# josl/kmerjs

Measured on AMD Instinct MI355X. Metric: k-mers/sec + distinct-kmers/sec, k=16 150bp synthetic FASTQ, 1/2/4/8 GPU, higher is better.
Workload: dtype u8; 1 GPU; C2: 10000000 synthetic 150bp reads per GPU, k=16, prefix 'ATGAC'; reads_per_gpu=10000000, mode=ordered (reference Map insertion order), k=16, prefix=ATGAC, bytes_per_gpu=3170000000, pipeline=off (steps in sequence), parallelism=dp1 (one GPU; no collective), backend=none

## Files before the change

### kmerjs_amd/csrc/kmer_kernels.hip

```cpp
#include "kmer_device.hpp"

#include <algorithm>
#include <cstring>

namespace kmerhip {

__device__ __forceinline__ uint32_t align4(uint32_t hi, uint32_t lo, uint32_t sel) {
    return __builtin_amdgcn_alignbyte(hi, lo, sel);
}

__device__ __forceinline__ void set_info(unsigned int *err, unsigned int bit) {
    if (!(__hip_atomic_load(err, __ATOMIC_RELAXED, __HIP_MEMORY_SCOPE_AGENT) & bit)) atomicOr(err, bit);
}

__device__ __forceinline__ uint32_t not_nl_bits(uint32_t x) {
    return ((x ^ 0x0A0A0A0Au) + 0x7F7F7F7Fu) & 0x80808080u;
}

__device__ __forceinline__ uint32_t not_nl_bits_xad(uint32_t x, uint32_t k0a, uint32_t k7f) {
    uint32_t r;
    asm("v_xad_u32 %0, %1, %2, %3" : "=v"(r) : "v"(x), "v"(k0a), "s"(k7f));
    return r & 0x80808080u;
}

__device__ __forceinline__ uint8_t comp_byte(uint8_t c) {
    return c == 'A' ? 'T' : c == 'T' ? 'A' : c == 'G' ? 'C' : c == 'C' ? 'G' : c;
}

__device__ __forceinline__ uint64_t lb_load(unsigned long long *p) {
    return __hip_atomic_load(p, __ATOMIC_RELAXED, __HIP_MEMORY_SCOPE_AGENT);
}
__device__ __forceinline__ void lb_store(unsigned long long *p, uint64_t v) {
    __hip_atomic_store(p, (unsigned long long)v, __ATOMIC_RELAXED, __HIP_MEMORY_SCOPE_AGENT);
}

constexpr uint32_t SPIN_LIMIT = 1u << 22;

template <bool SUM>
__device__ uint64_t look_back(unsigned long long *words, uint32_t tile, unsigned int *err) {
    const int lane = threadIdx.x & 63;
    uint64_t acc = 0;
    int64_t top = (int64_t)tile - 1;
    uint32_t spins = 0;
    while (true) {
        int64_t idx = top - lane;
        uint64_t v = 0;
        bool valid = idx >= 0;
        while (true) {
            v = valid ? lb_load(words + idx) : LB_INC;
            bool ready = (v >> 62) != 0;
            if (__all(ready)) break;
            if (++spins > SPIN_LIMIT) {
                if (lane == 0) atomicOr(err, ERR_LOOKBACK_TIMEOUT);
                return acc;
            }
            __builtin_amdgcn_s_sleep(1);
        }
        const uint64_t val = valid ? (v & LB_VAL) : 0;
        const bool inc = (v >> 62) == 2;
        if (SUM) {
            unsigned long long incmask = __ballot(inc);
            int stop = incmask ? __ffsll((long long)incmask) - 1 : 64;
            uint64_t contrib = lane <= stop ? val : 0;
            for (int d = 32; d >= 1; d >>= 1) contrib += __shfl_xor(contrib, d);
            acc += contrib;
            if (incmask) return acc;
        } else {
            unsigned long long hit = __ballot(inc || val != 0);
            if (hit) {
                int stop = __ffsll((long long)hit) - 1;
                return __shfl(val, stop);
            }
        }
        top -= 64;
    }
}

struct TileShared {
    uint32_t tpre[TPB + 1];
    uint32_t wsum[TPB / 64];
    int32_t last_thr;
    uint32_t tile;
    uint64_t line_base;
    uint64_t lnl_before;
    uint64_t lnl_tile;
    int32_t lastpos;
    uint32_t nh;
    uint32_t qn;
    uint32_t more;
    uint32_t q[1024];
};

__device__ __forceinline__ uint32_t nl_before_in_thread(const uint8_t *buf, int thr, int q) {
    const uint32_t *lw = (const uint32_t *)(buf + FH + 64 * thr);
    int n = q - 64 * thr;
    uint32_t c = 0;
#pragma unroll 1
    for (int i = 0; i < 16 && n > 0; ++i, n -= 4) {
        uint32_t z = nl_flags(lw[i]);
        if (n < 4) z &= (1u << (8 * n)) - 1u;
        c += __popc(z);
    }
    return c;
}

__device__ __forceinline__ uint32_t lds_word(const uint8_t *buf, int p) {
    const int a = FH + p;
    const uint32_t *w = (const uint32_t *)(buf + (a & ~3));
    return align4(w[1], w[0], (uint32_t)(a & 3));
}


__device__ __forceinline__ uint64_t revcomp_code(uint64_t x, uint32_t k) {
    x = ~x;
    x = ((x >> 2) & 0x3333333333333333ull) | ((x & 0x3333333333333333ull) << 2);
    x = ((x >> 4) & 0x0F0F0F0F0F0F0F0Full) | ((x & 0x0F0F0F0F0F0F0F0Full) << 4);
    x = __builtin_bswap64(x);
// ... 729 lines not shown
                                                uint32_t *lk, bool *lvalid_out, uint64_t *key_hi) {
    const uint32_t t = r.tile;
    const uint32_t strand = (r.qm >> 14) & 1u;
    const bool exotic = (r.qm >> 15) & 1u;
    const bool lvalid = (r.qm >> 16) & 1u;
    const int q = (int)(r.qm & 0x3FFFu);
    const int s0 = strand ? q + (int)a.plen - (int)a.k : q;
    const uint64_t tile_abs = a.abs_offset + (uint64_t)t * TILE;
    const uint64_t li = pos_lines + tb.cnt + r.c_local;
    const uint64_t lstart = lvalid ? tile_abs + r.lstart : tb.lnl;
    const uint64_t sabs = tile_abs + (uint64_t)(int64_t)s0;
    uint64_t rel = sabs - lstart;
    const bool seq = (li & 3) == 1;
    const uint64_t maxrel = (1ull << a.pbits) - 1ull;
    if (rel > maxrel) {
        if (seq) atomicOr(a.err, ERR_LINE_TOO_LONG);
        rel = maxrel;
    }
    if (li >> (63 - a.pbits)) atomicOr(a.err, ERR_LINE_TOO_LONG);
    const uint64_t order = (li << (a.pbits + 1)) | ((uint64_t)strand << a.pbits) | (strand ? maxrel - rel : rel);
    *order_out = order;
    const uint32_t sp = (uint32_t)(s0 + 64);
    *lk = (r.c_local << 17) | (strand << 16) | (strand ? 0xFFFFu - sp : sp);
    *lvalid_out = lvalid;
    uint64_t key = a.invalid_key;
    *key_hi = a.wide ? a.invalid_key : 0;
    if (a.wide) key = 0;
    if (seq) {
        if (a.packed && !exotic) {
            if (a.k > 32) {
                uint64_t h = code_hi, l = r.code;
                if (strand) revcomp_code128(code_hi, r.code, a.k, &h, &l);
                key = l & a.smask;
                *key_hi = h & a.smask_hi;
            } else {
                key = (strand ? revcomp_code(r.code, a.k) : r.code) & a.smask;
            }
        } else {
            append_record(a.recs, a.rec_count, a.rec_cap, a.err, order, (uint64_t)t * TILE + (uint64_t)(int64_t)s0, a.k,
                          strand);
        }
    }
    return key;
}

__device__ __forceinline__ void place_hit(const HitArgs &a, uint64_t slot, bool cross, uint64_t xi, uint64_t key,
                                          uint64_t key_hi, uint64_t order) {
    if (!cross) {
        if (slot >= a.rcap) {
            atomicOr(a.err, ERR_OVF_OVERFLOW);
            return;
        }
        if (a.rkey32) a.rkey32[slot] = (uint32_t)key;
        else a.rkey[slot] = key;
        if (a.wide) a.rkeyh[slot] = key_hi;
        a.rord[slot] = order;
    } else if (xi < a.xcap) {
        a.xord[xi] = order;
        a.xslot[xi] = (uint32_t)slot;
        if (a.wide) {
            a.xkey[xi] = xi;
            a.xkeyl[xi] = key;
            a.xkeyh[xi] = key_hi;
        } else {
            a.xkey[xi] = key;
        }
    } else {
        atomicOr(a.err, ERR_CROSS_OVERFLOW);
    }
}

constexpr uint32_t HTPW = 4;
constexpr uint32_t HENT = HTPW * HMAX;
template <bool WIDE>
__global__ __launch_bounds__(256) void hit_kernel(HitArgs a) {
    __shared__ uint32_t s_lk[4][HENT];
    __shared__ uint8_t s_x[4][HENT];
    __shared__ uint64_t s_key[4][HENT];
    __shared__ uint64_t s_ord[4][HENT];
    __shared__ uint64_t s_keyh[WIDE ? 4 : 1][WIDE ? HENT : 1];
    const uint32_t wid = threadIdx.x >> 6, lane = threadIdx.x & 63;
    const uint32_t t0 = __builtin_amdgcn_readfirstlane((blockIdx.x * 4 + wid) * HTPW);
    if (t0 >= a.n_tiles) return;
    const unsigned long long ovf = *a.ovf_count;
    const uint64_t pos_lines = a.pos->lines;
    TileSum ts[HTPW], tb[HTPW];
#pragma unroll
    for (uint32_t u = 0; u < HTPW; ++u) {
        const uint32_t t = min(t0 + u, a.n_tiles - 1);
        ts[u] = a.tsum[t];
        tb[u] = a.tscan[t];
    }
    if (ovf > a.ovf_cap) return;
    uint32_t off[HTPW + 1];
    off[0] = 0;
#pragma unroll
    for (uint32_t u = 0; u < HTPW; ++u) off[u + 1] = off[u] + (t0 + u < a.n_tiles ? min(ts[u].nh, (uint32_t)HMAX) : 0u);
    const uint32_t total = off[HTPW];
    for (uint32_t e0 = 0; e0 < total; e0 += 64) {
        const uint32_t e = e0 + lane;
        if (e < total) {
            uint32_t u = 0;
#pragma unroll
            for (uint32_t v = 1; v < HTPW; ++v) u += e >= off[v] ? 1u : 0u;
            const uint32_t i = e - off[u];
            TileSum tsu = ts[0], tbu = tb[0];
#pragma unroll
            for (uint32_t v = 1; v < HTPW; ++v)
                if (u == v) {
                    tsu = ts[v];
                    tbu = tb[v];
                }
            const uint64_t hslot = (uint64_t)(t0 + u) * HMAX + i;
            const HitRec r = a.hits[hslot];
            uint64_t order, kh;
            uint32_t lk;
            bool lvalid;
            const uint64_t key = resolve_hit(a, pos_lines, r, a.k > 32 ? a.hits_hi[hslot] : 0, tbu, &order, &lk, &lvalid,
                                             &kh);
            s_lk[wid][e] = lk;
            s_x[wid][e] = (tsu.nh > (uint32_t)HMAX || !lvalid || r.c_local == (uint32_t)tsu.cnt) ? 1 : 0;
            s_key[wid][e] = key;
            if (WIDE) s_keyh[WIDE ? wid : 0][WIDE ? e : 0] = kh;
            s_ord[wid][e] = order;
        }
    }
    if (!a.packed) return;
    __builtin_amdgcn_fence(__ATOMIC_RELEASE, "workgroup");
    __builtin_amdgcn_wave_barrier();
    for (uint32_t e0 = 0; e0 < total; e0 += 64) {
        const uint32_t e = e0 + lane;
        if (e >= total) continue;
        uint32_t u = 0;
#pragma unroll
        for (uint32_t v = 1; v < HTPW; ++v) u += e >= off[v] ? 1u : 0u;
        uint32_t lo = off[0], hi = off[1], nh = ts[0].nh;
        uint64_t hb = tb[0].nh, xb = tb[0].nx;
#pragma unroll
        for (uint32_t v = 1; v < HTPW; ++v)
            if (u == v) {
                lo = off[v];
                hi = off[v + 1];
                nh = ts[v].nh;
                hb = tb[v].nh;
                xb = tb[v].nx;
            }
        const uint32_t i = e - lo;
        const bool cross = s_x[wid][e] != 0;
        uint32_t rank = i, xr = i;
        if (nh <= (uint32_t)HMAX) {
            const uint32_t lk = s_lk[wid][e];
            rank = 0;
            xr = 0;
            for (uint32_t j = lo; j < hi; ++j) {
                const uint32_t less = s_lk[wid][j] < lk ? 1u : 0u;
                rank += less;
                xr += less & (uint32_t)s_x[wid][j];
            }
        }
        place_hit(a, a.out_base + hb + rank, cross, a.xbase + xb + xr, s_key[wid][e],
                  WIDE ? s_keyh[WIDE ? wid : 0][WIDE ? e : 0] : 0, s_ord[wid][e]);
    }
}

__global__ __launch_bounds__(256) void hit_overflow_kernel(HitArgs a) {
    const uint64_t n = *a.ovf_count <= a.ovf_cap ? *a.ovf_count : 0;
    for (uint64_t i = (uint64_t)blockIdx.x * blockDim.x + threadIdx.x; i < n; i += (uint64_t)gridDim.x * blockDim.x) {
        const HitRec r = a.ovf[i];
        const TileSum tb = a.tscan[r.tile];
        uint64_t order, kh;
        uint32_t lk;
        bool lvalid;
        const uint64_t key = resolve_hit(a, a.pos->lines, r, a.k > 32 ? a.ovf_hi[i] : 0, tb, &order, &lk, &lvalid, &kh);
        if (!a.packed) continue;
        const uint32_t ord = r.qm >> 17;
        place_hit(a, a.out_base + tb.nh + ord, true, a.xbase + tb.nx + ord, key, kh, order);
    }
    __shared__ bool last;
    __syncthreads();
    if (threadIdx.x == 0) {
        __threadfence();
        last = atomicAdd(a.ticket, 1u) == gridDim.x - 1;
    }
    __syncthreads();
    if (!last || threadIdx.x != 0) return;
    __threadfence();
    const uint32_t nt = a.n_tiles;
    StreamPos *pos = (StreamPos *)a.pos;
    pos->lines += a.tscan[nt - 1].cnt + a.tsum[nt - 1].cnt;
    pos->ends_open = (a.len > 0 && a.data[a.len - 1] != '\n') ? 1 : 0;
    *a.ends_open = pos->ends_open;
    *a.chunk_hits = a.tscan[nt - 1].nh + a.tsum[nt - 1].nh;
    *a.chunk_cross = a.tscan[nt - 1].nx + a.tsum[nt - 1].nx;
    *a.ticket = 0;
    if (a.stamp) a.stamp[STAMP_FEED_END] = wall_clock64();
    const uint64_t errw = __hip_atomic_load(a.scal + 5, __ATOMIC_RELAXED, __HIP_MEMORY_SCOPE_AGENT);
    *a.cross_go = ((uint32_t)errw & CROSS_HOST_BITS) ? 0u : 1u;
    __threadfence();
    if (a.host_out) {
        for (int i = 0; i < 8; ++i)
            a.host_out[i] = i == 5 ? errw : __hip_atomic_load(a.scal + i, __ATOMIC_RELAXED, __HIP_MEMORY_SCOPE_AGENT);
        if (a.stamp)
            for (int i = 0; i <= (int)STAMP_FEED_END; ++i)
                a.host_out[TAIL_STAMP + i] = __hip_atomic_load(a.stamp + i, __ATOMIC_RELAXED, __HIP_MEMORY_SCOPE_AGENT);
        __threadfence_system();
        __hip_atomic_store(a.host_out + 9, a.seq, __ATOMIC_RELEASE, __HIP_MEMORY_SCOPE_SYSTEM);
    }
}

__device__ __forceinline__ TileSum ts_shfl_up(const TileSum &v, int d) {
    TileSum r;
    r.cnt = (uint64_t)__shfl_up((unsigned long long)v.cnt, d);
    r.nh = (uint32_t)__shfl_up((int)v.nh, d);
    r.nx = (uint32_t)__shfl_up((int)v.nx, d);
    r.lnl = (uint64_t)__shfl_up((unsigned long long)v.lnl, d);
    return r;
}
__device__ __forceinline__ TileSum ts_zero() {
    TileSum z;
    z.cnt = 0;
    z.nh = 0;
    z.nx = 0;
    z.lnl = 0;
    return z;
}
__device__ __forceinline__ TileSum ts_wave_scan(TileSum v) {
    const int lane = threadIdx.x & 63;
#pragma unroll
    for (int d = 1; d < 64; d <<= 1) {
        const TileSum o = ts_shfl_up(v, d);
        if (lane >= d) v = tile_sum_op(o, v);
    }
    return v;
}
__device__ __forceinline__ TileSum ts_block_scan(TileSum v, TileSum *total) {
    __shared__ TileSum wsum[4];
    const int lane = threadIdx.x & 63, wid = threadIdx.x >> 6;
    const TileSum incl = ts_wave_scan(v);
    if (lane == 63) wsum[wid] = incl;
    __syncthreads();
    TileSum pre = ts_zero(), tot = ts_zero();
#pragma unroll
    for (int w = 0; w < 4; ++w) {
        if (w < wid) pre = tile_sum_op(pre, wsum[w]);
        tot = tile_sum_op(tot, wsum[w]);
    }
    __syncthreads();
    *total = tot;
    const TileSum ex = ts_shfl_up(incl, 1);
    return lane == 0 ? pre : tile_sum_op(pre, ex);
}

__global__ __launch_bounds__(256) void tile_reduce_kernel(const TileSum *in, uint32_t n, TileSum *bsum,
                                                          uint64_t *stamp) {
    stamp_now(stamp, STAMP_SCAN_END);
    const uint32_t base = blockIdx.x * TSCAN_BLOCK;
    TileSum v = ts_zero();
#pragma unroll
    for (uint32_t i = 0; i < TSCAN_BLOCK / 256; ++i) {
        const uint32_t t = base + i * 256 + threadIdx.x;
        if (t < n) v = tile_sum_op(v, in[t]);
    }
    TileSum tot;
    (void)ts_block_scan(v, &tot);
    if (threadIdx.x == 0) bsum[blockIdx.x] = tot;
}

__global__ __launch_bounds__(256) void tile_scan_kernel(const TileSum *in, uint32_t n, const TileSum *bsum,
                                                        uint32_t bsum_scanned, TileSum init, TileSum *out) {
    const uint32_t b = blockIdx.x;
    TileSum pre;
    if (bsum_scanned) {
        pre = tile_sum_op(init, bsum[b]);
    } else {
        TileSum v = ts_zero();
        for (uint32_t j = threadIdx.x; j < b; j += 256) v = tile_sum_op(v, bsum[j]);
        TileSum tot;
        (void)ts_block_scan(v, &tot);
        pre = tile_sum_op(init, tot);
    }
    const uint32_t t0 = b * TSCAN_BLOCK + threadIdx.x * 4;
    TileSum x[4];
    TileSum acc = ts_zero();
#pragma unroll
    for (int i = 0; i < 4; ++i) {
        x[i] = t0 + i < n ? in[t0 + i] : ts_zero();
        acc = tile_sum_op(acc, x[i]);
    }
    TileSum tot;
// ... 999 lines not shown
        HeadRec v;
        v.key = 0;
        v.count = 0;
        if (k != invalid_key && (i == 0 || skey[i - 1] != k)) {
            const uint64_t e = group_end(skey, i, n, k);
            uint64_t cnt = e - i;
            if (rcnt) {
                cnt = 0;
                for (uint64_t j = i; j < e; ++j) cnt += rcnt[srank[j]];
            }
            v.key = k;
            v.count = cnt;
        }
        const uint32_t r = srank[i];
        hrec[r] = v;
        hcnt[r] = v.count ? 1u : 0u;
    }
}

template <typename K>
__global__ __launch_bounds__(256) void heads_sparse_kernel(const K *skey, const uint32_t *srank, uint64_t n,
                                                           K invalid_key, uint32_t *hcnt) {
    for (uint64_t i = (uint64_t)blockIdx.x * blockDim.x + threadIdx.x; i < n; i += (uint64_t)gridDim.x * blockDim.x) {
        const K k = skey[i];
        const bool dp = i > 0 && skey[i - 1] == k;
        const bool dn = i + 1 < n && skey[i + 1] == k;
        if (k != invalid_key && !dp && !dn) continue;
        uint32_t v = 0;
        if (k != invalid_key && !dp) v = (uint32_t)(group_end(skey, i, n, k) - i);
        hcnt[srank[i]] = v;
    }
}

__global__ __launch_bounds__(256) void gather_u64_kernel(const uint64_t *src, const uint32_t *idx, uint64_t n,
                                                         uint64_t *dst) {
    for (uint64_t i = (uint64_t)blockIdx.x * blockDim.x + threadIdx.x; i < n; i += (uint64_t)gridDim.x * blockDim.x)
        dst[i] = src[idx[i]];
}

__global__ __launch_bounds__(256) void cross_wide_fix_kernel(const uint32_t *xslot, uint64_t n, const uint64_t *xkeyl,
                                                             const uint64_t *xkeyh, uint64_t *rkey, uint64_t *rkeyh) {
    for (uint64_t i = (uint64_t)blockIdx.x * blockDim.x + threadIdx.x; i < n; i += (uint64_t)gridDim.x * blockDim.x) {
        const uint32_t sl = xslot[i];
        const uint64_t x = rkey[sl];
        rkey[sl] = xkeyl[x];
        rkeyh[sl] = xkeyh[x];
    }
}

__global__ __launch_bounds__(256) void heads_wide_kernel(const uint64_t *shi, const uint64_t *slo,
                                                         const uint32_t *srank, uint64_t n, uint64_t invalid_hi,
                                                         uint32_t *hcnt) {
    for (uint64_t i = (uint64_t)blockIdx.x * blockDim.x + threadIdx.x; i < n; i += (uint64_t)gridDim.x * blockDim.x) {
        const uint64_t h = shi[i], l = slo[i];
        const bool dp = i > 0 && shi[i - 1] == h && slo[i - 1] == l;
        const bool dn = i + 1 < n && shi[i + 1] == h && slo[i + 1] == l;
        const bool inv = h == invalid_hi;
        if (!inv && !dp && !dn) continue;
        uint32_t v = 0;
        if (!inv && !dp) {
            uint64_t e = i + 1;
            while (e < n && shi[e] == h && slo[e] == l) ++e;
            v = (uint32_t)(e - i);
        }
        hcnt[srank[i]] = v;
    }
}

constexpr uint32_t BKT_EPB = 4096;

__global__ __launch_bounds__(256) void bucket_hist_kernel(const uint32_t *key, uint64_t n, uint32_t invalid,
                                                          uint32_t shift, uint32_t nb, uint32_t nblk,
                                                          uint32_t *H, uint32_t *hcnt, uint64_t *stamp) {
    stamp_now(stamp, STAMP_FINISH_START);
    __shared__ uint32_t hist[BKT_MAX];
    for (uint32_t b = threadIdx.x; b < nb; b += 256) hist[b] = 0;
    __syncthreads();
    const uint64_t base = (uint64_t)blockIdx.x * BKT_EPB;
    for (uint32_t j = 4 * threadIdx.x; j < BKT_EPB; j += 4 * 256) {
        const uint64_t i = base + j;
        if (i + 4 <= n) *(uint4 *)(hcnt + i) = make_uint4(0, 0, 0, 0);
        else for (uint64_t t = i; t < n; ++t) hcnt[t] = 0;
    }
#pragma unroll 4
    for (uint32_t j = threadIdx.x; j < BKT_EPB; j += 256) {
        const uint64_t i = base + j;
        if (i < n) {
            const uint32_t k = key[i];
            if (k != invalid) atomicAdd(&hist[k >> shift], 1u);
        }
    }
    __syncthreads();
    for (uint32_t b = threadIdx.x; b < nb; b += 256) H[(uint64_t)b * nblk + blockIdx.x] = hist[b];
}

__global__ __launch_bounds__(256) void bucket_offsets_kernel(const uint32_t *H, uint32_t nb, uint32_t nblk,
                                                             uint32_t *Hs, uint32_t *btot, uint32_t *bbase,
                                                             unsigned int *ticket) {
    __shared__ uint32_t ws[4];
    __shared__ bool last;
    const uint32_t b = blockIdx.x, tid = threadIdx.x, lane = tid & 63, wid = tid >> 6;
    const uint32_t per = (nblk + 255) / 256, j0 = tid * per, j1 = min(j0 + per, nblk);
    const uint32_t *row = H + (uint64_t)b * nblk;
    uint32_t sum = 0;
    for (uint32_t j = j0; j < j1; ++j) sum += row[j];
    const uint32_t incl = wave_incl_sum(sum);
    if (lane == 63) ws[wid] = incl;
    __syncthreads();
    uint32_t pre = incl - sum;
    for (uint32_t w = 0; w < wid; ++w) pre += ws[w];
    uint32_t *out = Hs + (uint64_t)b * nblk;
    for (uint32_t j = j0; j < j1; ++j) {
        const uint32_t v = row[j];
        out[j] = pre;
        pre += v;
    }
    if (tid == 0) {
        __hip_atomic_store(btot + b, ws[0] + ws[1] + ws[2] + ws[3], __ATOMIC_RELAXED, __HIP_MEMORY_SCOPE_AGENT);
        last = __hip_atomic_fetch_add(ticket, 1u, __ATOMIC_ACQ_REL, __HIP_MEMORY_SCOPE_AGENT) == nb - 1;
    }
    __syncthreads();
    if (!last) return;
    uint32_t v[BKT_MAX / 256], s = 0;
#pragma unroll
    for (uint32_t u = 0; u < BKT_MAX / 256; ++u) {
        const uint32_t q = tid * (BKT_MAX / 256) + u;
        v[u] = q < nb ? __hip_atomic_fetch_add(btot + q, 0u, __ATOMIC_RELAXED, __HIP_MEMORY_SCOPE_AGENT) : 0u;
        s += v[u];
    }
    const uint32_t inc2 = wave_incl_sum(s);
    __syncthreads();
    if (lane == 63) ws[wid] = inc2;
    __syncthreads();
    uint32_t p = inc2 - s;
    for (uint32_t w = 0; w < wid; ++w) p += ws[w];
#pragma unroll
    for (uint32_t u = 0; u < BKT_MAX / 256; ++u) {
        const uint32_t q = tid * (BKT_MAX / 256) + u;
        if (q < nb) bbase[q] = p;
        p += v[u];
    }
    if (tid == 255) bbase[nb] = p;
    if (tid == 0) *ticket = 0;
}

__global__ __launch_bounds__(256) void bucket_scatter_kernel(const uint32_t *key, uint64_t n, uint32_t invalid,
                                                             uint32_t shift, uint32_t nb, uint32_t nblk,
                                                             const uint32_t *Hs, const uint32_t *bbase, uint16_t *pkey,
                                                             uint32_t *prank) {
    __shared__ uint32_t cnt[BKT_MAX];
    __shared__ uint32_t skey[BKT_EPB];
    __shared__ uint32_t srank[BKT_EPB];
    __shared__ uint32_t wtot[4];
    for (uint32_t b = threadIdx.x; b < nb; b += 256) cnt[b] = 0;
    __syncthreads();
    const uint64_t base = (uint64_t)blockIdx.x * BKT_EPB;
    uint32_t kk[BKT_EPB / 256], li[BKT_EPB / 256];
#pragma unroll
    for (uint32_t u = 0; u < BKT_EPB / 256; ++u) {
        const uint64_t i = base + u * 256 + threadIdx.x;
        kk[u] = i < n ? key[i] : invalid;
        li[u] = kk[u] != invalid ? atomicAdd(&cnt[kk[u] >> shift], 1u) : 0u;
    }
    __syncthreads();
    uint32_t loc[BKT_MAX / 256], sum = 0;
#pragma unroll
    for (uint32_t u = 0; u < BKT_MAX / 256; ++u) {
        const uint32_t b = threadIdx.x * (BKT_MAX / 256) + u;
        loc[u] = b < nb ? cnt[b] : 0u;
        sum += loc[u];
    }
    uint32_t gpos[BKT_MAX / 256];
#pragma unroll
    for (uint32_t u = 0; u < BKT_MAX / 256; ++u) {
        const uint32_t b = threadIdx.x * (BKT_MAX / 256) + u;
        gpos[u] = b < nb && loc[u] ? bbase[b] + Hs[(uint64_t)b * nblk + blockIdx.x] : 0u;
    }
    const uint32_t incl = wave_incl_sum(sum);
    if ((threadIdx.x & 63) == 63) wtot[threadIdx.x >> 6] = incl;
    __syncthreads();
    uint32_t pre = incl - sum;
    for (uint32_t w = 0; w < (threadIdx.x >> 6); ++w) pre += wtot[w];
    uint32_t lst[BKT_MAX / 256];
#pragma unroll
    for (uint32_t u = 0; u < BKT_MAX / 256; ++u) {
        const uint32_t b = threadIdx.x * (BKT_MAX / 256) + u;
        lst[u] = pre;
        if (b < nb) cnt[b] = pre;
        pre += loc[u];
    }
    const uint32_t valid = wtot[0] + wtot[1] + wtot[2] + wtot[3];
    __syncthreads();
#pragma unroll
    for (uint32_t u = 0; u < BKT_EPB / 256; ++u) {
        if (kk[u] != invalid) {
            const uint32_t p = cnt[kk[u] >> shift] + li[u];
            skey[p] = kk[u];
            srank[p] = (uint32_t)(base + u * 256 + threadIdx.x);
        }
    }
    __syncthreads();
#pragma unroll
    for (uint32_t u = 0; u < BKT_MAX / 256; ++u) {
        const uint32_t b = threadIdx.x * (BKT_MAX / 256) + u;
        if (b < nb && loc[u]) cnt[b] = gpos[u] - lst[u];
    }
    __syncthreads();
    const uint32_t lo_mask = (1u << shift) - 1u;
    for (uint32_t e = threadIdx.x; e < valid; e += 256) {
        const uint32_t k = skey[e], b = k >> shift;
        const uint32_t pos = cnt[b] + e;
        pkey[pos] = (uint16_t)(k & lo_mask);
        prank[pos] = srank[e];
    }
}

constexpr uint32_t BKT_SKIP = 0x80000000u;

__global__ __launch_bounds__(256) void bucket_onepass_kernel(const uint32_t *key, uint64_t n, uint32_t invalid,
                                                             uint32_t shift, uint32_t nb, uint32_t cap, uint32_t *cur,
                                                             uint16_t *pkey, uint32_t *prank, uint32_t *hcnt,
                                                             unsigned int *err, uint64_t *stamp) {
    stamp_now(stamp, STAMP_FINISH_START);
    __shared__ uint32_t cnt[BKT_MAX];
    __shared__ uint32_t skey[BKT_EPB];
    __shared__ uint32_t srank[BKT_EPB];
    __shared__ uint32_t wtot[4];
    for (uint32_t b = threadIdx.x; b < nb; b += 256) cnt[b] = 0;
    __syncthreads();
    const uint64_t base = (uint64_t)blockIdx.x * BKT_EPB;
    for (uint32_t j = 4 * threadIdx.x; j < BKT_EPB; j += 4 * 256) {
        const uint64_t i = base + j;
        if (i + 4 <= n) *(uint4 *)(hcnt + i) = make_uint4(0, 0, 0, 0);
        else for (uint64_t t = i; t < n; ++t) hcnt[t] = 0;
    }
    uint32_t kk[BKT_EPB / 256], li[BKT_EPB / 256];
#pragma unroll
    for (uint32_t u = 0; u < BKT_EPB / 256; ++u) {
        const uint64_t i = base + u * 256 + threadIdx.x;
        kk[u] = i < n ? key[i] : invalid;
        li[u] = kk[u] != invalid ? atomicAdd(&cnt[kk[u] >> shift], 1u) : 0u;
    }
    __syncthreads();
    uint32_t loc[BKT_MAX / 256], sum = 0;
#pragma unroll
    for (uint32_t u = 0; u < BKT_MAX / 256; ++u) {
        const uint32_t b = threadIdx.x * (BKT_MAX / 256) + u;
        loc[u] = b < nb ? cnt[b] : 0u;
        sum += loc[u];
    }
    uint32_t gpos[BKT_MAX / 256];
#pragma unroll
    for (uint32_t u = 0; u < BKT_MAX / 256; ++u) {
        const uint32_t b = threadIdx.x * (BKT_MAX / 256) + u;
        gpos[u] = b < nb && loc[u] ? atomicAdd(cur + (uint64_t)b * BKT_CUR_STRIDE, loc[u]) : 0u;
    }
    const uint32_t incl = wave_incl_sum(sum);
    if ((threadIdx.x & 63) == 63) wtot[threadIdx.x >> 6] = incl;
    __syncthreads();
    uint32_t pre = incl - sum;
    for (uint32_t w = 0; w < (threadIdx.x >> 6); ++w) pre += wtot[w];
    uint32_t lst[BKT_MAX / 256];
#pragma unroll
    for (uint32_t u = 0; u < BKT_MAX / 256; ++u) {
        const uint32_t b = threadIdx.x * (BKT_MAX / 256) + u;
        lst[u] = pre;
        if (b < nb) cnt[b] = pre;
        pre += loc[u];
    }
    const uint32_t valid = wtot[0] + wtot[1] + wtot[2] + wtot[3];
    __syncthreads();
#pragma unroll
    for (uint32_t u = 0; u < BKT_EPB / 256; ++u) {
        if (kk[u] != invalid) {
            const uint32_t p = cnt[kk[u] >> shift] + li[u];
            skey[p] = kk[u];
            srank[p] = (uint32_t)(base + u * 256 + threadIdx.x);
        }
    }
    __syncthreads();
    bool over = false;
#pragma unroll
    for (uint32_t u = 0; u < BKT_MAX / 256; ++u) {
        const uint32_t b = threadIdx.x * (BKT_MAX / 256) + u;
        if (b < nb && loc[u]) {
            const bool fits = (uint64_t)gpos[u] + loc[u] <= cap;
            cnt[b] = fits ? b * cap + gpos[u] - lst[u] : BKT_SKIP;
            over |= !fits;
        }
    }
    if (over) atomicOr(err, ERR_BKT_CAP);
    __syncthreads();
    const uint32_t lo_mask = (1u << shift) - 1u;
    for (uint32_t e = threadIdx.x; e < valid; e += 256) {
        const uint32_t k = skey[e], b = k >> shift;
        const uint32_t c = cnt[b];
        if (c == BKT_SKIP) continue;
        const uint32_t pos = c + e;
        pkey[pos] = (uint16_t)(k & lo_mask);
        prank[pos] = srank[e];
    }
}

__global__ __launch_bounds__(1024) void bucket_heads_kernel(const uint16_t *pkey, const uint32_t *prank,
                                                            const uint32_t *bbase, uint32_t shift, uint32_t *hcnt,
                                                            uint32_t *cur, uint32_t cap, uint64_t n,
                                                            unsigned int *err) {
    __shared__ uint32_t minr[1u << BKT_LOW];
    __shared__ uint32_t cnt[1u << BKT_LOW];
    __shared__ uint32_t s_tot;
    const uint32_t b = blockIdx.x, nk = 1u << shift;
    if (cur && threadIdx.x == 0) s_tot = atomicExch(cur + (uint64_t)b * BKT_CUR_STRIDE, 0u);
    for (uint32_t j = threadIdx.x; j < nk; j += blockDim.x) {
        minr[j] = 0xFFFFFFFFu;
        cnt[j] = 0;
    }
    __syncthreads();
    uint32_t lo, hi;
    if (cur) {
        lo = b * cap;
        hi = s_tot <= cap ? lo + s_tot : lo;
    } else {
        lo = bbase[b];
        hi = bbase[b + 1];
    }
    constexpr uint32_t U = 16;
    for (uint32_t e0 = lo; e0 < hi; e0 += U * 1024) {
        uint32_t j[U], r[U];
#pragma unroll
        for (uint32_t u = 0; u < U; ++u) {
            const uint32_t e = e0 + u * 1024 + threadIdx.x;
            j[u] = e < hi ? pkey[e] & (nk - 1u) : 0u;
            r[u] = e < hi ? prank[e] : 0u;
        }
#pragma unroll
        for (uint32_t u = 0; u < U; ++u) {
            if (e0 + u * 1024 + threadIdx.x < hi) {
                atomicMin(&minr[j[u]], r[u]);
                atomicAdd(&cnt[j[u]], 1u);
            }
        }
    }
    __syncthreads();
    for (uint32_t j = threadIdx.x; j < nk; j += blockDim.x) {
        const uint32_t c = cnt[j];
        if (c) {
            const uint32_t r = minr[j];
            if (r < n) hcnt[r] = c;
            else atomicOr(err, ERR_BKT_RANK);
        }
    }
}

constexpr uint32_t EMIT_RPB = 1024;
__global__ __launch_bounds__(256) void head_count_kernel(const uint32_t *hcnt, uint64_t n, uint32_t *ecnt) {
    __shared__ uint32_t ws[4];
    const uint64_t r0 = (uint64_t)blockIdx.x * EMIT_RPB + 4 * threadIdx.x;
    uint32_t c = 0;
    if (r0 + 4 <= n) {
        const uint4 v = *(const uint4 *)(hcnt + r0);
        c = (v.x != 0) + (v.y != 0) + (v.z != 0) + (v.w != 0);
    } else {
        for (uint64_t r = r0; r < n; ++r) c += hcnt[r] != 0;
    }
    c = wave_incl_sum(c);
    if ((threadIdx.x & 63) == 63) ws[threadIdx.x >> 6] = c;
    __syncthreads();
    if (threadIdx.x == 0) ecnt[blockIdx.x] = ws[0] + ws[1] + ws[2] + ws[3];
}

__global__ __launch_bounds__(256) void emit_kernel(EmitArgs a) {
    __shared__ __attribute__((aligned(16))) uint8_t kbuf[256 * KMAX_TILE];
    __shared__ uint32_t s_w[EMIT_RPB / 256][4];
    __shared__ uint64_t s_pre;
    __shared__ uint32_t s_wp[4];
    const uint64_t n = a.n;
    const uint32_t k = a.k, plen = a.plen;
    const bool staged = !a.partial && (k & 3);
    const int tid = threadIdx.x, lane = tid & 63, wid = tid >> 6;
    const uint64_t rb = (uint64_t)blockIdx.x * EMIT_RPB;
    constexpr int NR = EMIT_RPB / 256;
    uint32_t hcr[NR];
    unsigned long long hm[NR];
#pragma unroll
    for (int i = 0; i < NR; ++i) {
        const uint64_t r = rb + 256 * i + tid;
        hcr[i] = r < n ? a.hcnt[r] : 0u;
        hm[i] = __ballot(hcr[i] != 0);
        if (lane == 0) s_w[i][wid] = (uint32_t)__popcll(hm[i]);
    }
    uint64_t ekey[NR], ecnt[NR], efirst[NR], ekeyh[NR];
#pragma unroll
    for (int i = 0; i < NR; ++i) {
        const uint64_t r = rb + 256 * i + tid;
        ekey[i] = ecnt[i] = efirst[i] = ekeyh[i] = 0;
        if (hcr[i]) {
            if (a.hrec) {
                const HeadRec v = a.hrec[r];
                ekey[i] = v.key;
                ecnt[i] = v.count;
            } else {
                ekey[i] = a.rkey32 ? (uint64_t)a.rkey32[r] : a.rkey64[r];
                if (a.rkeyh) ekeyh[i] = a.rkeyh[r];
                ecnt[i] = hcr[i];
            }
            efirst[i] = a.rord[r];
        }
    }
    if (a.epre) {
        if (tid == 0) s_pre = a.epre[blockIdx.x];
    } else {
        uint32_t p = 0;
        for (uint32_t j = tid; j < blockIdx.x; j += 256) p += a.ecnt[j];
        p = wave_incl_sum(p);
        if (lane == 63) s_wp[wid] = p;
    }
    __syncthreads();
    if (!a.epre && tid == 0) s_pre = (uint64_t)s_wp[0] + s_wp[1] + s_wp[2] + s_wp[3];
    __syncthreads();
    uint64_t o0 = s_pre;
#pragma unroll
    for (int i = 0; i < NR; ++i) {
        const uint64_t r = rb + 256 * i + tid;
        if (rb + 256 * i >= n) break;
        uint32_t before = 0, rt = 0;
#pragma unroll
        for (int w = 0; w < 4; ++w) {
            before += w < wid ? s_w[i][w] : 0u;
            rt += s_w[i][w];
        }
        const uint32_t hc = hcr[i];
        const uint32_t f = hc ? 1u : 0u;
        const uint64_t o64 = o0 + before +
                             __builtin_amdgcn_mbcnt_hi((uint32_t)(hm[i] >> 32), __builtin_amdgcn_mbcnt_lo((uint32_t)hm[i], 0u));
        const uint64_t oend = o0 + rt;
        if (r == n - 1) {
            *a.nuniq = o64 + f;
            if (a.host_out) {
                a.host_out[TAIL_ERR] = __hip_atomic_load(a.err, __ATOMIC_RELAXED, __HIP_MEMORY_SCOPE_AGENT);
                if (a.stamp) a.host_out[TAIL_FIN_START] = a.stamp[STAMP_FINISH_START];
            }
            if (a.nuniq_host) {
                *a.nuniq_host = o64 + f;
                __threadfence_system();
            }
        }
        const uint64_t o = o64;
        if (f) {
            const uint64_t key = ekey[i], cnt = ecnt[i], keyh = ekeyh[i], first = efirst[i];
            if (a.partial) {
                a.ukey[o] = key;
                Agg v;
                v.first = first;
                v.count = cnt;
                a.uval[o] = v;
            } else {
                a.cnt_out[o] = cnt;
                a.first_out[o] = first;
                uint8_t *out = staged ? kbuf + (o - o0) * k : a.keys_out + o * k;
                const uint32_t nw = (k + 3) / 4;
                uint32_t w0 = 0, w1 = 0, w2 = 0;
                for (int w = 0; w < KMAX_TILE / 4; ++w) {
                    if ((uint32_t)w >= nw) break;
                    uint32_t v = 0;
#pragma unroll
                    for (int j = 0; j < 4; ++j) {
                        const uint32_t pos = 4 * w + j;
                        uint32_t ch = 0;
                        if (pos < plen) {
                            ch = a.P[pos];
                        } else if (pos < k) {
                            const uint32_t sh = 2 * (k - 1 - pos);
                            const uint32_t b = (uint32_t)(sh < 64 ? key >> sh : keyh >> (sh - 64)) & 3u;
                            ch = (0x54474341u >> (8 * b)) & 0xFFu;
                        }
                        v |= ch << (8 * j);
                    }
                    if (k == 16) {
                        if (w == 0) w0 = v;
                        else if (w == 1) w1 = v;
                        else if (w == 2) w2 = v;
                        else *(uint4 *)out = make_uint4(w0, w1, w2, v);
                    } else if ((k & 3) == 0) {
                        *(uint32_t *)(out + 4 * w) = v;
                    } else {
                        for (uint32_t b = 4 * w; b < k && b < 4 * (uint32_t)w + 4; ++b)
                            out[b] = (uint8_t)(v >> (8 * (b & 3)));
                    }
                }
            }
        }
        if (staged) {
            __syncthreads();
            const uint64_t g0 = (uint64_t)o0 * k, g1 = (uint64_t)oend * k;
            const uint64_t a0 = (g0 + 3) & ~3ull, a1 = g1 & ~3ull;
            if (a0 >= a1) {
                for (uint64_t g = g0 + threadIdx.x; g < g1; g += 256) a.keys_out[g] = kbuf[g - g0];
            } else {
                if (threadIdx.x < a0 - g0) a.keys_out[g0 + threadIdx.x] = kbuf[threadIdx.x];
                if (threadIdx.x < g1 - a1) a.keys_out[a1 + threadIdx.x] = kbuf[a1 - g0 + threadIdx.x];
                const uint32_t sh = (uint32_t)(a0 - g0);
                for (uint64_t g = a0 + 4 * threadIdx.x; g < a1; g += 4 * 256) {
                    const uint32_t l = (uint32_t)(g - g0);
                    const uint32_t v = sh == 0 ? *(const uint32_t *)(kbuf + l)
                                               : (uint32_t)kbuf[l] | ((uint32_t)kbuf[l + 1] << 8) |
                                                     ((uint32_t)kbuf[l + 2] << 16) | ((uint32_t)kbuf[l + 3] << 24);
                    *(uint32_t *)(a.keys_out + g) = v;
                }
            }
            __syncthreads();
        }
        o0 = oend;
    }
    if (a.host_out && a.stamp && blockIdx.x == gridDim.x - 1 && tid == 0) {
        a.host_out[TAIL_FIN_END] = wall_clock64();
        __threadfence_system();
    }
}

__global__ __launch_bounds__(256) void merge_prep_kernel(const uint64_t *keys, const Agg *vals, uint64_t n,
                                                         uint64_t *rkey, uint32_t *rkey32, uint64_t *rord,
                                                         uint64_t *rcnt, uint32_t *ridx) {
    for (uint64_t i = (uint64_t)blockIdx.x * blockDim.x + threadIdx.x; i < n; i += (uint64_t)gridDim.x * blockDim.x) {
        const Agg v = vals[i];
        put_key(rkey, rkey32, i, keys[i]);
        rord[i] = v.first;
        rcnt[i] = v.count;
        ridx[i] = (uint32_t)i;
    }
}

constexpr uint32_t XP_EPB = 4096;
// ... 436 lines not shown
    return hipGetLastError();
}

hipError_t launch_gather_u64(const uint64_t *src, const uint32_t *idx, uint64_t n, uint64_t *dst, hipStream_t s) {
    if (n) hipLaunchKernelGGL(gather_u64_kernel, dim3(grid_for(n)), dim3(256), 0, s, src, idx, n, dst);
    return hipGetLastError();
}
hipError_t launch_cross_wide_fix(const uint32_t *xslot, uint64_t n, const uint64_t *xkeyl, const uint64_t *xkeyh,
                                 uint64_t *rkey, uint64_t *rkeyh, hipStream_t s) {
    if (n) hipLaunchKernelGGL(cross_wide_fix_kernel, dim3(grid_for(n)), dim3(256), 0, s, xslot, n, xkeyl, xkeyh, rkey,
                              rkeyh);
    return hipGetLastError();
}
hipError_t launch_heads_wide(const uint64_t *shi, const uint64_t *slo, const uint32_t *srank, uint64_t n,
                             uint64_t invalid_hi, uint32_t *hcnt, hipStream_t s) {
    if (n) hipLaunchKernelGGL(heads_wide_kernel, dim3(grid_for(n)), dim3(256), 0, s, shi, slo, srank, n, invalid_hi,
                              hcnt);
    return hipGetLastError();
}
hipError_t launch_heads(const uint64_t *skey, const uint32_t *srank, uint64_t n, uint64_t invalid_key,
                        const uint64_t *rcnt, HeadRec *hrec, uint32_t *hcnt, hipStream_t s) {
    if (n)
        hipLaunchKernelGGL(heads_kernel<uint64_t>, dim3(grid_for(n)), dim3(256), 0, s, skey, srank, n, invalid_key, rcnt,
                           hrec, hcnt);
    return hipGetLastError();
}
hipError_t launch_heads_sparse(const uint64_t *skey64, const uint32_t *skey32, const uint32_t *srank, uint64_t n,
                               uint64_t invalid_key, uint32_t *hcnt, hipStream_t s) {
    if (!n) return hipSuccess;
    if (skey32)
        hipLaunchKernelGGL(heads_sparse_kernel<uint32_t>, dim3(grid_for(n)), dim3(256), 0, s, skey32, srank, n,
                           (uint32_t)invalid_key, hcnt);
    else
        hipLaunchKernelGGL(heads_sparse_kernel<uint64_t>, dim3(grid_for(n)), dim3(256), 0, s, skey64, srank, n,
                           invalid_key, hcnt);
    return hipGetLastError();
}
hipError_t launch_heads32(const uint32_t *skey, const uint32_t *srank, uint64_t n, uint32_t invalid_key,
                          const uint64_t *rcnt, HeadRec *hrec, uint32_t *hcnt, hipStream_t s) {
    if (n)
        hipLaunchKernelGGL(heads_kernel<uint32_t>, dim3(grid_for(n)), dim3(256), 0, s, skey, srank, n, invalid_key, rcnt,
                           hrec, hcnt);
    return hipGetLastError();
}
hipError_t launch_bucket_hist(const uint32_t *key, uint64_t n, uint32_t invalid, uint32_t shift, uint32_t nb,
                              uint32_t nblk, uint32_t *H, uint32_t *hcnt, uint64_t *stamp, hipStream_t s) {
    hipLaunchKernelGGL(bucket_hist_kernel, dim3(nblk), dim3(256), 0, s, key, n, invalid, shift, nb, nblk, H, hcnt,
                       stamp);
    return hipGetLastError();
}
hipError_t launch_bucket_offsets(const uint32_t *H, uint32_t nb, uint32_t nblk, uint32_t *Hs, uint32_t *btot,
                                 uint32_t *bbase, unsigned int *ticket, hipStream_t s) {
    hipLaunchKernelGGL(bucket_offsets_kernel, dim3(nb), dim3(256), 0, s, H, nb, nblk, Hs, btot, bbase, ticket);
    return hipGetLastError();
}
hipError_t launch_bucket_scatter(const uint32_t *key, uint64_t n, uint32_t invalid, uint32_t shift, uint32_t nb,
                                 uint32_t nblk, const uint32_t *Hs, const uint32_t *bbase, uint16_t *pkey,
                                 uint32_t *prank, hipStream_t s) {
    hipLaunchKernelGGL(bucket_scatter_kernel, dim3(nblk), dim3(256), 0, s, key, n, invalid, shift, nb, nblk, Hs, bbase,
                       pkey, prank);
    return hipGetLastError();
}
hipError_t launch_bucket_onepass(const uint32_t *key, uint64_t n, uint32_t invalid, uint32_t shift, uint32_t nb,
                                 uint32_t nblk, uint32_t cap, uint32_t *cur, uint16_t *pkey, uint32_t *prank,
                                 uint32_t *hcnt, unsigned int *err, uint64_t *stamp, hipStream_t s) {
    if (nb == 0 || nb > BKT_MAX || (uint64_t)nb * cap > 0x7FFFFFFFull) return hipErrorInvalidValue;
    hipLaunchKernelGGL(bucket_onepass_kernel, dim3(nblk), dim3(256), 0, s, key, n, invalid, shift, nb, cap, cur, pkey,
                       prank, hcnt, err, stamp);
    return hipGetLastError();
}
hipError_t launch_bucket_heads(const uint16_t *pkey, const uint32_t *prank, const uint32_t *bbase, uint32_t nb,
                               uint32_t shift, uint32_t *hcnt, uint32_t *cur, uint32_t cap, uint64_t n,
                               unsigned int *err, hipStream_t s) {
    hipLaunchKernelGGL(bucket_heads_kernel, dim3(nb), dim3(1024), 0, s, pkey, prank, bbase, shift, hcnt, cur, cap, n,
                       err);
    return hipGetLastError();
}
uint64_t emit_blocks(uint64_t n) { return (n + EMIT_RPB - 1) / EMIT_RPB; }
hipError_t launch_head_count(const uint32_t *hcnt, uint64_t n, uint32_t *ecnt, hipStream_t s) {
    if (n) hipLaunchKernelGGL(head_count_kernel, dim3((uint32_t)emit_blocks(n)), dim3(256), 0, s, hcnt, n, ecnt);
    return hipGetLastError();
}
hipError_t launch_emit(const EmitArgs &a, hipStream_t s) {
    if (a.n) hipLaunchKernelGGL(emit_kernel, dim3((uint32_t)emit_blocks(a.n)), dim3(256), 0, s, a);
    return hipGetLastError();
}
hipError_t launch_merge_prep(const uint64_t *keys, const Agg *vals, uint64_t n, uint64_t *rkey, uint32_t *rkey32,
                             uint64_t *rord, uint64_t *rcnt, uint32_t *ridx, hipStream_t s) {
    if (n)
        hipLaunchKernelGGL(merge_prep_kernel, dim3(grid_for(n)), dim3(256), 0, s, keys, vals, n, rkey, rkey32, rord, rcnt,
                           ridx);
    return hipGetLastError();
}
hipError_t launch_xpart_hist(const uint64_t *rkey, const uint32_t *rkey32, uint64_t n, uint64_t invalid,
                             uint32_t kbits, uint32_t world, uint32_t nblk, uint32_t *H, hipStream_t s) {
    if (world == 0 || world > XP_MAXW || nblk == 0) return hipErrorInvalidValue;
    hipLaunchKernelGGL(xpart_hist_kernel, dim3(nblk), dim3(256), 0, s, rkey, rkey32, n, invalid, kbits, world, nblk, H);
    return hipGetLastError();
}
hipError_t launch_xpart_scatter(const uint64_t *rkey, const uint32_t *rkey32, const uint64_t *rord, uint64_t n,
                                uint64_t invalid, uint32_t kbits, uint32_t world, uint32_t nblk, const uint32_t *H,
                                const uint32_t *Hs, XHit *out, uint64_t *counts, hipStream_t s) {
    if (world == 0 || world > XP_MAXW || nblk == 0) return hipErrorInvalidValue;
    hipLaunchKernelGGL(xpart_scatter_kernel, dim3(nblk), dim3(256), 0, s, rkey, rkey32, rord, n, invalid, kbits, world,
                       nblk, Hs, out);
    hipLaunchKernelGGL(xpart_counts_kernel, dim3(1), dim3(256), 0, s, H, Hs, world, nblk, counts);
    return hipGetLastError();
}
hipError_t launch_xprep(const XHit *x, uint64_t n, uint64_t *rkey, uint32_t *rkey32, uint64_t *rord, uint32_t *ridx,
                        hipStream_t s) {
    if (n) hipLaunchKernelGGL(xprep_kernel, dim3(grid_for(n)), dim3(256), 0, s, x, n, rkey, rkey32, rord, ridx);
    return hipGetLastError();
}
hipError_t launch_gather_records(const Record *recs, uint64_t stride, uint64_t n, const uint8_t *data,
                                 uint8_t *out, hipStream_t s) {
    if (n == 0) return hipSuccess;
    uint64_t blocks = (n + 255) / 256;
    if (blocks > 8192) blocks = 8192;
    hipLaunchKernelGGL(gather_records_kernel, dim3((uint32_t)blocks), dim3(256), 0, s, recs, stride, n, data, out);
    return hipGetLastError();
}

hipError_t launch_nl_write(const uint8_t *data, uint64_t len, uint32_t n_tiles, const uint64_t *tbase, uint64_t *nl,
                           hipStream_t s) {
    hipLaunchKernelGGL(nl_write_kernel, dim3(n_tiles), dim3(256), 0, s, data, len, tbase, nl);
    return hipGetLastError();
}
hipError_t launch_nl_slots(const uint8_t *data, uint64_t len, uint32_t n_tiles, uint32_t cap, uint16_t *slots,
                          uint32_t *tcount, unsigned int *err, hipStream_t s) {
    hipLaunchKernelGGL(nl_slots_kernel, dim3(n_tiles), dim3(256), 0, s, data, len, cap, slots, tcount, err);
    return hipGetLastError();
}
hipError_t launch_seq_lines_slots(const uint16_t *slots, const uint32_t *tcount, const uint64_t *tbase,
                                  uint32_t n_tiles, uint32_t cap, uint64_t len, uint64_t li0, uint64_t first,
                                  uint64_t n_nl, uint64_t n_seq, uint32_t k, uint32_t step, SeqLine *lines,
                                  uint64_t *wcount, unsigned int *err, uint64_t maxrel, hipStream_t s) {
    if (!n_seq) return hipSuccess;
    hipLaunchKernelGGL(seq_lines_slots_kernel, dim3((n_tiles + 3) / 4), dim3(256), 0, s, slots, tcount, tbase,
                       n_tiles, cap, len, li0, first, n_nl, n_seq, k, step, lines, wcount, err, maxrel);
    return hipGetLastError();
}
hipError_t launch_seq_lines(const uint64_t *nl, uint64_t n_nl, uint64_t len, uint64_t li0, uint64_t n_seq, uint32_t k,
                            uint32_t step, SeqLine *lines, uint64_t *wcount, unsigned int *err, uint64_t maxrel,
                            hipStream_t s) {
    if (n_seq)
        hipLaunchKernelGGL(seq_lines_kernel, dim3(grid_for(n_seq)), dim3(256), 0, s, nl, n_nl, len, li0, n_seq, k, step,
                           lines, wcount, err, maxrel);
    return hipGetLastError();
}
hipError_t launch_pos_after(StreamPos *pos, uint64_t lines, const uint8_t *data, uint64_t len,
                            unsigned long long *ends_open, hipStream_t s) {
    hipLaunchKernelGGL(pos_after_kernel, dim3(1), dim3(64), 0, s, pos, lines, data, len, ends_open);
    return hipGetLastError();
}
hipError_t launch_windows_packed(const WinArgs &a, hipStream_t s) {
    if (a.n_lines) {
        const uint64_t cap = a.block_lines ? 65536 : 262144;
        const uint64_t w = a.n_lines < cap ? a.n_lines : cap;
        hipLaunchKernelGGL(windows_packed_kernel, dim3((uint32_t)(a.block_lines ? w : (w + 3) / 4)), dim3(256), 0, s, a);
    }
    return hipGetLastError();
}
hipError_t launch_synth_fastq(uint8_t *out, uint64_t seed, uint64_t first_read, uint64_t n_reads, hipStream_t s) {
    const uint64_t chunks = (n_reads * 317 + 15) / 16;
    uint64_t blocks = (chunks + 255) / 256;
    if (blocks > 65536) blocks = 65536;
    if (blocks == 0) return hipSuccess;
// ... 6 lines not shown
```

Baseline: 4208 billion k-mers/s.

## Batch unconditional loads, template emit routes, and parallelize tail writeback

Several kernels (bucket hist/scatter, heads, emit) now issue all global loads up front with clamped indices, so they no longer sit behind per-element branches and more memory requests can be in flight before the atomics. emit_kernel is templated on the key source, which removes runtime pointer checks, and it prefetches the earlier block counts into registers. hit_kernel adds empty asm constraints to keep uniform values in scalar registers. The last-block tail in the feed kernel now copies scalars and stamps to host memory with one wave instead of a serial loop in a single thread. The clamped loads do redundant reads at the edges, and the register-pinning hints could raise register pressure.

```diff
diff --git a/kmerjs_amd/csrc/kmer_kernels.hip b/kmerjs_amd/csrc/kmer_kernels.hip
--- a/kmerjs_amd/csrc/kmer_kernels.hip
+++ b/kmerjs_amd/csrc/kmer_kernels.hip
@@ -33,6 +33,16 @@
 __device__ __forceinline__ void lb_store(unsigned long long *p, uint64_t v) {
     __hip_atomic_store(p, (unsigned long long)v, __ATOMIC_RELAXED, __HIP_MEMORY_SCOPE_AGENT);
 }
+
+template <typename I>
+__device__ __forceinline__ I clamp_idx(I i, I n) {
+    return i < n ? i : n - 1;
+}
+__device__ __forceinline__ void sgpr_pin(uint32_t &v) { asm volatile("" : "+s"(v)); }
+__device__ __forceinline__ void sgpr_pin(uint64_t &v) { asm volatile("" : "+s"(v)); }
+__device__ __forceinline__ void sgpr_pin(unsigned long long &v) { asm volatile("" : "+s"(v)); }
+template <typename T>
+__device__ __forceinline__ void sgpr_use(T v) { asm volatile("" : : "s"(v)); }
 
 constexpr uint32_t SPIN_LIMIT = 1u << 22;
 
@@ -928,8 +938,8 @@
     const uint32_t wid = threadIdx.x >> 6, lane = threadIdx.x & 63;
     const uint32_t t0 = __builtin_amdgcn_readfirstlane((blockIdx.x * 4 + wid) * HTPW);
     if (t0 >= a.n_tiles) return;
-    const unsigned long long ovf = *a.ovf_count;
-    const uint64_t pos_lines = a.pos->lines;
+    unsigned long long ovf = *a.ovf_count;
+    uint64_t pos_lines = a.pos->lines;
     TileSum ts[HTPW], tb[HTPW];
 #pragma unroll
     for (uint32_t u = 0; u < HTPW; ++u) {
@@ -937,7 +947,20 @@
         ts[u] = a.tsum[t];
         tb[u] = a.tscan[t];
     }
+    sgpr_use(a.k), sgpr_use(a.plen), sgpr_use(a.packed), sgpr_use(a.pbits), sgpr_use(a.wide), sgpr_use(a.ovf_cap);
+    sgpr_use(a.abs_offset), sgpr_use(a.smask), sgpr_use(a.smask_hi), sgpr_use(a.invalid_key), sgpr_use(a.err);
+    sgpr_use(a.hits), sgpr_use(a.hits_hi), sgpr_use(a.recs), sgpr_use(a.rec_count), sgpr_use(a.rec_cap);
+    sgpr_pin(ovf);
+    sgpr_pin(pos_lines);
+#pragma unroll
+    for (uint32_t u = 0; u < HTPW; ++u) {
+        sgpr_pin(ts[u].cnt), sgpr_pin(ts[u].nh);
+        sgpr_pin(tb[u].cnt), sgpr_pin(tb[u].nh), sgpr_pin(tb[u].nx), sgpr_pin(tb[u].lnl);
+    }
     if (ovf > a.ovf_cap) return;
+    const HitRec *const hits = a.hits;
+    const uint64_t *const hits_hi = a.hits_hi;
+    const bool has_hi = a.k > 32;
     uint32_t off[HTPW + 1];
     off[0] = 0;
 #pragma unroll
@@ -958,12 +981,12 @@
                     tbu = tb[v];
                 }
             const uint64_t hslot = (uint64_t)(t0 + u) * HMAX + i;
-            const HitRec r = a.hits[hslot];
+            const HitRec r = hits[hslot];
+            const uint64_t code_hi = has_hi ? hits_hi[hslot] : 0;
             uint64_t order, kh;
             uint32_t lk;
             bool lvalid;
-            const uint64_t key = resolve_hit(a, pos_lines, r, a.k > 32 ? a.hits_hi[hslot] : 0, tbu, &order, &lk, &lvalid,
-                                             &kh);
+            const uint64_t key = resolve_hit(a, pos_lines, r, code_hi, tbu, &order, &lk, &lvalid, &kh);
             s_lk[wid][e] = lk;
             s_x[wid][e] = (tsu.nh > (uint32_t)HMAX || !lvalid || r.c_local == (uint32_t)tsu.cnt) ? 1 : 0;
             s_key[wid][e] = key;
@@ -1029,28 +1052,39 @@
         last = atomicAdd(a.ticket, 1u) == gridDim.x - 1;
     }
     __syncthreads();
-    if (!last || threadIdx.x != 0) return;
-    __threadfence();
-    const uint32_t nt = a.n_tiles;
-    StreamPos *pos = (StreamPos *)a.pos;
-    pos->lines += a.tscan[nt - 1].cnt + a.tsum[nt - 1].cnt;
-    pos->ends_open = (a.len > 0 && a.data[a.len - 1] != '\n') ? 1 : 0;
-    *a.ends_open = pos->ends_open;
-    *a.chunk_hits = a.tscan[nt - 1].nh + a.tsum[nt - 1].nh;
-    *a.chunk_cross = a.tscan[nt - 1].nx + a.tsum[nt - 1].nx;
-    *a.ticket = 0;
-    if (a.stamp) a.stamp[STAMP_FEED_END] = wall_clock64();
-    const uint64_t errw = __hip_atomic_load(a.scal + 5, __ATOMIC_RELAXED, __HIP_MEMORY_SCOPE_AGENT);
-    *a.cross_go = ((uint32_t)errw & CROSS_HOST_BITS) ? 0u : 1u;
+    if (!last) return;
+    if (threadIdx.x == 0) {
+        __threadfence();
+        const uint32_t nt = a.n_tiles;
+        StreamPos *pos = (StreamPos *)a.pos;
+        const TileSum lb = a.tscan[nt - 1], ls = a.tsum[nt - 1];
+        const uint64_t open = (a.len > 0 && a.data[a.len - 1] != '\n') ? 1 : 0;
+        pos->lines += lb.cnt + ls.cnt;
+        pos->ends_open = open;
+        *a.ends_open = open;
+        *a.chunk_hits = lb.nh + ls.nh;
+        *a.chunk_cross = lb.nx + ls.nx;
+        *a.ticket = 0;
+        if (a.stamp) a.stamp[STAMP_FEED_END] = wall_clock64();
+        __threadfence();
+    }
+    __syncthreads();
+    if (threadIdx.x >= 64) return;
+    const uint32_t lane = threadIdx.x;
+    const uint32_t nw = 8u + (a.stamp ? (uint32_t)STAMP_FEED_END + 1u : 0u);
+    uint64_t v = 0;
+    if (lane < nw && (a.host_out || lane == 5)) {
+        const uint64_t *src = lane < 8 ? a.scal + lane : a.stamp + (lane - 8);
+        v = __hip_atomic_load(src, __ATOMIC_RELAXED, __HIP_MEMORY_SCOPE_AGENT);
+    }
+    const uint32_t errw = (uint32_t)__builtin_amdgcn_readlane((int)(uint32_t)v, 5);
+    if (lane == 0) *a.cross_go = (errw & CROSS_HOST_BITS) ? 0u : 1u;
     __threadfence();
     if (a.host_out) {
-        for (int i = 0; i < 8; ++i)
-            a.host_out[i] = i == 5 ? errw : __hip_atomic_load(a.scal + i, __ATOMIC_RELAXED, __HIP_MEMORY_SCOPE_AGENT);
-        if (a.stamp)
-            for (int i = 0; i <= (int)STAMP_FEED_END; ++i)
-                a.host_out[TAIL_STAMP + i] = __hip_atomic_load(a.stamp + i, __ATOMIC_RELAXED, __HIP_MEMORY_SCOPE_AGENT);
+        if (lane < nw) a.host_out[lane < 8 ? lane : TAIL_STAMP + (lane - 8)] = v;
         __threadfence_system();
-        __hip_atomic_store(a.host_out + 9, a.seq, __ATOMIC_RELEASE, __HIP_MEMORY_SCOPE_SYSTEM);
+        __builtin_amdgcn_wave_barrier();
+        if (lane == 0) __hip_atomic_store(a.host_out + 9, a.seq, __ATOMIC_RELEASE, __HIP_MEMORY_SCOPE_SYSTEM);
     }
 }
 
@@ -2216,14 +2250,16 @@
         if (i + 4 <= n) *(uint4 *)(hcnt + i) = make_uint4(0, 0, 0, 0);
         else for (uint64_t t = i; t < n; ++t) hcnt[t] = 0;
     }
-#pragma unroll 4
-    for (uint32_t j = threadIdx.x; j < BKT_EPB; j += 256) {
-        const uint64_t i = base + j;
-        if (i < n) {
-            const uint32_t k = key[i];
-            if (k != invalid) atomicAdd(&hist[k >> shift], 1u);
-        }
-    }
+    uint32_t kk[BKT_EPB / 256];
+#pragma unroll
+    for (uint32_t u = 0; u < BKT_EPB / 256; ++u) {
+        const uint64_t i = base + u * 256 + threadIdx.x;
+        const uint32_t v = key[clamp_idx(i, n)];
+        kk[u] = i < n ? v : invalid;
+    }
+#pragma unroll
+    for (uint32_t u = 0; u < BKT_EPB / 256; ++u)
+        if (kk[u] != invalid) atomicAdd(&hist[kk[u] >> shift], 1u);
     __syncthreads();
     for (uint32_t b = threadIdx.x; b < nb; b += 256) H[(uint64_t)b * nblk + blockIdx.x] = hist[b];
 }
@@ -2293,9 +2329,12 @@
 #pragma unroll
     for (uint32_t u = 0; u < BKT_EPB / 256; ++u) {
         const uint64_t i = base + u * 256 + threadIdx.x;
-        kk[u] = i < n ? key[i] : invalid;
+        const uint32_t v = key[clamp_idx(i, n)];
+        kk[u] = i < n ? v : invalid;
+    }
+#pragma unroll
+    for (uint32_t u = 0; u < BKT_EPB / 256; ++u)
         li[u] = kk[u] != invalid ? atomicAdd(&cnt[kk[u] >> shift], 1u) : 0u;
-    }
     __syncthreads();
     uint32_t loc[BKT_MAX / 256], sum = 0;
 #pragma unroll
@@ -2372,9 +2411,12 @@
 #pragma unroll
     for (uint32_t u = 0; u < BKT_EPB / 256; ++u) {
         const uint64_t i = base + u * 256 + threadIdx.x;
-        kk[u] = i < n ? key[i] : invalid;
+        const uint32_t v = key[clamp_idx(i, n)];
+        kk[u] = i < n ? v : invalid;
+    }
+#pragma unroll
+    for (uint32_t u = 0; u < BKT_EPB / 256; ++u)
         li[u] = kk[u] != invalid ? atomicAdd(&cnt[kk[u] >> shift], 1u) : 0u;
-    }
     __syncthreads();
     uint32_t loc[BKT_MAX / 256], sum = 0;
 #pragma unroll
@@ -2464,8 +2506,9 @@
 #pragma unroll
         for (uint32_t u = 0; u < U; ++u) {
             const uint32_t e = e0 + u * 1024 + threadIdx.x;
-            j[u] = e < hi ? pkey[e] & (nk - 1u) : 0u;
-            r[u] = e < hi ? prank[e] : 0u;
+            const uint32_t ec = e < hi ? e : hi - 1;
+            j[u] = pkey[ec] & (nk - 1u);
+            r[u] = prank[ec];
         }
 #pragma unroll
         for (uint32_t u = 0; u < U; ++u) {
@@ -2503,6 +2546,8 @@
     if (threadIdx.x == 0) ecnt[blockIdx.x] = ws[0] + ws[1] + ws[2] + ws[3];
 }
 
+enum : int { EMIT_HREC = 0, EMIT_KEY32 = 1, EMIT_KEY64 = 2, EMIT_KEY128 = 3 };
+template <int ROUTE>
 __global__ __launch_bounds__(256) void emit_kernel(EmitArgs a) {
     __shared__ __attribute__((aligned(16))) uint8_t kbuf[256 * KMAX_TILE];
     __shared__ uint32_t s_w[EMIT_RPB / 256][4];
@@ -2514,38 +2559,72 @@
     const int tid = threadIdx.x, lane = tid & 63, wid = tid >> 6;
     const uint64_t rb = (uint64_t)blockIdx.x * EMIT_RPB;
     constexpr int NR = EMIT_RPB / 256;
+    const uint32_t lastr = (uint32_t)(n - rb < EMIT_RPB ? n - rb : (uint64_t)EMIT_RPB) - 1u;
+    uint32_t rc[NR];
+#pragma unroll
+    for (int i = 0; i < NR; ++i) rc[i] = min((uint32_t)(256 * i + tid), lastr);
     uint32_t hcr[NR];
+    {
+        const uint32_t *hcnt = a.hcnt + rb;
+#pragma unroll
+        for (int i = 0; i < NR; ++i) hcr[i] = hcnt[rc[i]];
+    }
+    uint64_t ekey[NR], eaux[NR], efirst[NR];
+#pragma unroll
+    for (int i = 0; i < NR; ++i) eaux[i] = 0;
+    if (ROUTE == EMIT_HREC) {
+        const HeadRec *hrec = a.hrec + rb;
+#pragma unroll
+        for (int i = 0; i < NR; ++i) {
+            const HeadRec v = hrec[rc[i]];
+            ekey[i] = v.key;
+            eaux[i] = v.count;
+        }
+    } else if (ROUTE == EMIT_KEY32) {
+        const uint32_t *rkey32 = a.rkey32 + rb;
+#pragma unroll
+        for (int i = 0; i < NR; ++i) ekey[i] = (uint64_t)rkey32[rc[i]];
+    } else {
+        const uint64_t *rkey64 = a.rkey64 + rb;
+#pragma unroll
+        for (int i = 0; i < NR; ++i) ekey[i] = rkey64[rc[i]];
+        if (ROUTE == EMIT_KEY128) {
+            const uint64_t *rkeyh = a.rkeyh + rb;
+#pragma unroll
+            for (int i = 0; i < NR; ++i) eaux[i] = rkeyh[rc[i]];
+        }
+    }
+    {
+        const uint64_t *rord = a.rord + rb;
+#pragma unroll
+        for (int i = 0; i < NR; ++i) efirst[i] = rord[rc[i]];
+    }
+    static_assert(EMIT_DIRECT_MAX <= 16 * 256, "emit_kernel sums at most 4,096 earlier counts");
+    const uint32_t nbk = blockIdx.x;
+    uint32_t pc[16];
+#pragma unroll
+    for (uint32_t q = 0; q < 16; ++q) pc[q] = 0;
+    if (!a.epre) {
+#pragma unroll
+        for (uint32_t b = 0; b < 4; ++b)
+            if (nbk > b * 1024) {
+#pragma unroll
+                for (uint32_t q = 4 * b; q < 4 * b + 4; ++q) pc[q] = a.ecnt[clamp_idx(q * 256 + tid, nbk)];
+            }
+    }
     unsigned long long hm[NR];
 #pragma unroll
     for (int i = 0; i < NR; ++i) {
-        const uint64_t r = rb + 256 * i + tid;
-        hcr[i] = r < n ? a.hcnt[r] : 0u;
+        if (rb + 256 * i + tid >= n) hcr[i] = 0;
         hm[i] = __ballot(hcr[i] != 0);
         if (lane == 0) s_w[i][wid] = (uint32_t)__popcll(hm[i]);
-    }
-    uint64_t ekey[NR], ecnt[NR], efirst[NR], ekeyh[NR];
-#pragma unroll
-    for (int i = 0; i < NR; ++i) {
-        const uint64_t r = rb + 256 * i + tid;
-        ekey[i] = ecnt[i] = efirst[i] = ekeyh[i] = 0;
-        if (hcr[i]) {
-            if (a.hrec) {
-                const HeadRec v = a.hrec[r];
-                ekey[i] = v.key;
-                ecnt[i] = v.count;
-            } else {
-                ekey[i] = a.rkey32 ? (uint64_t)a.rkey32[r] : a.rkey64[r];
-                if (a.rkeyh) ekeyh[i] = a.rkeyh[r];
-                ecnt[i] = hcr[i];
-            }
-            efirst[i] = a.rord[r];
-        }
     }
     if (a.epre) {
         if (tid == 0) s_pre = a.epre[blockIdx.x];
     } else {
         uint32_t p = 0;
-        for (uint32_t j = tid; j < blockIdx.x; j += 256) p += a.ecnt[j];
+#pragma unroll
+        for (uint32_t q = 0; q < 16; ++q) p += q * 256 + tid < nbk ? pc[q] : 0u;
         p = wave_incl_sum(p);
         if (lane == 63) s_wp[wid] = p;
     }
@@ -2581,7 +2660,9 @@
         }
         const uint64_t o = o64;
         if (f) {
-            const uint64_t key = ekey[i], cnt = ecnt[i], keyh = ekeyh[i], first = efirst[i];
+            const uint64_t key = ekey[i], first = efirst[i];
+            const uint64_t cnt = ROUTE == EMIT_HREC ? eaux[i] : (uint64_t)hc;
+            const uint64_t keyh = ROUTE == EMIT_KEY128 ? eaux[i] : 0;
             if (a.partial) {
                 a.ukey[o] = key;
                 Agg v;
@@ -3184,7 +3265,12 @@
     return hipGetLastError();
 }
 hipError_t launch_emit(const EmitArgs &a, hipStream_t s) {
-    if (a.n) hipLaunchKernelGGL(emit_kernel, dim3((uint32_t)emit_blocks(a.n)), dim3(256), 0, s, a);
+    if (!a.n) return hipGetLastError();
+    const dim3 grid((uint32_t)emit_blocks(a.n));
+    if (a.hrec) hipLaunchKernelGGL(emit_kernel<EMIT_HREC>, grid, dim3(256), 0, s, a);
+    else if (a.rkey32) hipLaunchKernelGGL(emit_kernel<EMIT_KEY32>, grid, dim3(256), 0, s, a);
+    else if (a.rkeyh) hipLaunchKernelGGL(emit_kernel<EMIT_KEY128>, grid, dim3(256), 0, s, a);
+    else hipLaunchKernelGGL(emit_kernel<EMIT_KEY64>, grid, dim3(256), 0, s, a);
     return hipGetLastError();
 }
 hipError_t launch_merge_prep(const uint64_t *keys, const Agg *vals, uint64_t n, uint64_t *rkey, uint32_t *rkey32,
```

Measured after the change: 4280 billion k-mers/s (median of 6 runs). Within noise of the previous version (+1.7%).
